# leaxer-ai/leaxer-qwen3-tts

Hardware: AMD Instinct MI355X
Metric: real-time factor (24 kHz audio sec / wall sec), Qwen3-TTS-0.6B (higher is better)
Workload: dtype bf16 weights, fp32 activations/accumulate (codec decoder: fp16 hi/lo split operands, fp32 accumulate)

## Files before the change

### leaxer-qwen3-tts_amd/csrc/q3_common.h

```cpp
#pragma once
#include <hip/hip_runtime.h>
#include <stdint.h>
#include <string>

#include "../../include/q3tts.h"

typedef uint16_t bf16_t;

#define Q3_HIP_CHECK(expr)                                                                         \
    do {                                                                                           \
        hipError_t _e = (expr);                                                                    \
        if (_e != hipSuccess) throw q3::Error(std::string(#expr) + ": " + hipGetErrorString(_e));  \
    } while (0)

namespace q3 {

struct Error {
    std::string msg;
    explicit Error(std::string m) : msg(std::move(m)) {}
};

const char* knob(const char* name);
struct KnobScope {
    bool on = false;
// ... 5 lines not shown
    uint32_t u;
    __builtin_memcpy(&u, &f, 4);
    u = (u + 0x7FFFu + ((u >> 16) & 1u)) >> 16;
    return (bf16_t)u;
}
inline float bf16_to_f32(bf16_t b) {
    uint32_t u = (uint32_t)b << 16;
    float f;
    __builtin_memcpy(&f, &u, 4);
    return f;
}


enum GemvEpi { EPI_STORE = 0, EPI_RESIDUAL = 1, EPI_SWIGLU = 2, EPI_BIAS = 3, EPI_BIAS_SILU = 4, EPI_SLAB = 5, EPI_SLAB2 = 6 };

struct GemvArgs {
    const bf16_t* W = nullptr;
    const bf16_t* W2 = nullptr;
    const float* x = nullptr;
    int ldx = 0;
    const float* gamma = nullptr;
    float eps = 0.f;
    float* xn_out = nullptr;
    int ld_xn = 0;
    const float* bias = nullptr;
    const float* res = nullptr;
    int ldres = 0;
    float* out = nullptr;
    int ldo = 0;
    int M = 0, N = 0, K = 0;
    int epi = EPI_STORE;
    bool nt = false;
    const float* po = nullptr;
    const float* pm = nullptr;
    const float* pl = nullptr;
    int pS = 0, pchunk = 0, pn_new = 1, pslot_offset = 0, pheads = 0, pd = 0;
    const int* ppos_dev = nullptr;
    int ppos_scalar = 0;
    const float* psum = nullptr;
    float* xmid = nullptr;
};
void launch_gemv(const GemvArgs& a, hipStream_t s);
bool gemv_fast_path(const GemvArgs& a);
bool gemv16_ok(const GemvArgs& a);
void launch_gemv16(const GemvArgs& a, hipStream_t s);
void launch_pack_mfma_b(const bf16_t* W, bf16_t* P, int N, int K, hipStream_t s);
size_t packed_mfma_b_elems(int N, int K);
void register_packed_weight(const bf16_t* W, const bf16_t* P);
void unregister_packed_weight(const bf16_t* W);
const bf16_t* find_packed_weight(const bf16_t* W);

struct AttnArgs {
    const float* qkv = nullptr;
    int ld_qkv = 0;
    const float* ssq_in = nullptr; int ssq_nt = 0, ssq_K = 0; float ssq_eps = 0.f;
// ... 116 lines not shown
    float* x_talk = nullptr;
    const float* trailing = nullptr;
    int max_trailing = 0;
    const float* tts_pad = nullptr;
    int32_t* codes = nullptr;
    int max_frames_cap = 0;
    int32_t* talker_pos = nullptr;
    bf16_t* pl_h = nullptr; bf16_t* pl_l = nullptr; int pl_ldp = 0;
    const float* gamma0 = nullptr;
    float* ssq_out = nullptr; int ssq_nt = 0;
    int pl_row_mul = 1, pl_row_add = 0;
    const float* lh = nullptr; int ld_lh = 0;
    unsigned* step_gen = nullptr;
};
void launch_sample(const SampleArgs& a, hipStream_t s);

void launch_gather_rows_bf16(const bf16_t* table, int H, const int64_t* ids_dev, int n, float* out, int ldo, hipStream_t s);
void launch_fill_synth(void* dst, int is_bf16, int64_t n, uint64_t key, float mean, float stddev, hipStream_t s);
void launch_copy_rows(const float* src, int lds, float* dst, int ldd, int rows, int cols, hipStream_t s);
void launch_copy_rows_masked(const float* src, int lds, float* dst, int ldd, int rows, int cols, const int* flags_dev, hipStream_t s);
void launch_bump_u32(unsigned* counter, hipStream_t s);
void launch_count_active(const SlotState* st, int nb, int32_t* out, hipStream_t s);

struct ConvArgs {
    const float* in = nullptr; int T_in = 0, C_in = 0;
    float* out = nullptr;      int T_out = 0, C_out = 0;
    const float* W = nullptr;
    const bf16_t* Wh = nullptr; const bf16_t* Wl = nullptr;
    float w_scale_inv = 1.0f;
    bool w_lo_zero = false, w2_lo_zero = false;
// ... 57 lines not shown
```

### leaxer-qwen3-tts_amd/csrc/q3_decode_kernels.hip

```cpp
#include "q3_common.h"
#include "q3_wave_sort.h"
#include <algorithm>

namespace q3 {

#ifdef Q3_SAMPLE_PROF
__device__ long long g_kernel_prof[32];
void sample_prof_read(long long* out) { (void)hipMemcpyFromSymbol(out, HIP_SYMBOL(g_kernel_prof), sizeof(long long) * 32); }
#define KP_MARK(k) do { if (blockIdx.x == 0 && blockIdx.y == 0 && blockIdx.z == 0 && threadIdx.x == 0) g_kernel_prof[k] = wall_clock64(); } while (0)
#else
#define KP_MARK(k) do { } while (0)
#endif

#define Q3_DPP_XOR1 0xB1
#define Q3_DPP_XOR2 0x4E
#define Q3_DPP_ROR4 0x124
#define Q3_DPP_ROR8 0x128
#define Q3_DPP_BCAST15 0x142
#define Q3_DPP_BCAST31 0x143
template <int CTRL, int ROW_MASK>
static __device__ __forceinline__ float dpp_f(float oldv, float v) {
    return __builtin_bit_cast(float, __builtin_amdgcn_update_dpp(__builtin_bit_cast(int, oldv), __builtin_bit_cast(int, v), CTRL, ROW_MASK, 0xF, false));
}
template <int CTRL, int ROW_MASK>
// ... 391 lines not shown
            if (EPI == EPI_SWIGLU) { s2 = wave_sum(s2); if (lane == m * RW + r) mine2 = s2; }
        }
    KP_MARK(11);
    if (lane < MT * RW) {
        const int m = lane / RW, r = lane % RW, n = n0 + r;
        if (m < M && n < N) {
            float o;
            if (EPI == EPI_STORE) o = mine;
            else if (EPI == EPI_RESIDUAL) o = epi_in + mine;
            else if (EPI == EPI_SWIGLU) o = silu_f(mine) * mine2;
            else if (EPI == EPI_BIAS) o = mine + epi_in;
            else o = silu_f(mine + epi_in);
            a.out[(size_t)m * a.ldo + n] = o;
        }
    }
}

static int gemv1_rw(const GemvArgs& a) {
    int rw = a.N / 1024;
    if (rw < 1) rw = 1;
    if (rw > 4) rw = 4;
    if (a.epi == EPI_SWIGLU && rw > 3) rw = 3;
    if (a.K > 3072 && rw > 2) rw = 2;
    return rw;
}
bool gemv_fast_path(const GemvArgs& a) {
    if (a.M < 1 || a.M > 2) return false;
    if (a.K != 1024 && a.K != 2048 && a.K != 3072 && !(a.K == 6144 && a.M == 1)) return false;
    if (a.ldx % 4 != 0 && !a.po) return false;
    const bool norm = a.gamma != nullptr, comb = a.po != nullptr;
// ... 37 lines not shown
    else if constexpr (NCH <= 6) {
        if (rw == 3) gemv1_launch<MT, NCH, 3>(a, grid, s);
        else gemv1_launch<MT, NCH, 4>(a, grid, s);
    } else throw Error("gemv: K = 6144 fast path takes at most 2 rows per wave");
}
template <int MT>
static void gemv1_nch(const GemvArgs& a, hipStream_t s) {
    if (a.K == 1024) gemv1_rwsel<MT, 2>(a, s);
    else if (a.K == 2048) gemv1_rwsel<MT, 4>(a, s);
    else if (a.K == 3072) gemv1_rwsel<MT, 6>(a, s);
    else if constexpr (MT == 1) gemv1_rwsel<1, 12>(a, s);
    else throw Error("gemv: K = 6144 fast path is single-row");
}

void launch_gemv(const GemvArgs& a0, hipStream_t s) {
    if (gemv_fast_path(a0)) {
        if (a0.M == 1) gemv1_nch<1>(a0, s); else gemv1_nch<2>(a0, s);
        return;
    }
    if (gemv16_ok(a0)) { launch_gemv16(a0, s); return; }
    if (a0.po) throw Error("gemv: attention-partials prologue needs the fast path (combine separately)");
    if (a0.K % 8 != 0 || a0.ldx % 4 != 0) throw Error("gemv: K must be a multiple of 8 and ldx of 4");
    if ((a0.epi == EPI_RESIDUAL || a0.epi == EPI_BIAS || a0.epi == EPI_BIAS_SILU) && a0.gamma) throw Error("gemv: norm+epilogue combination not built");
    if (a0.M <= 0 || a0.N <= 0) return;
    for (int m0 = 0; m0 < a0.M; m0 += 8) {
        GemvArgs a = a0;
        a.M = a0.M - m0 < 8 ? a0.M - m0 : 8;
        a.x = a0.x + (size_t)m0 * a0.ldx;
        a.out = a0.out + (size_t)m0 * a0.ldo;
        if (a0.res) a.res = a0.res + (size_t)m0 * a0.ldres;
// ... 1808 lines not shown
    return draw_small_exact(ei, id0, havei != 0, nk, top_p, u, lane, sb);
}

static __device__ __forceinline__ float kth_largest_of_lanes(float v, int k) {
    const int lane = threadIdx.x & 63;
    const float sorted = wave_sort_desc(v, lane);
    const int r = __builtin_amdgcn_readfirstlane(k) - 1;
    return lane_bcast(sorted, r < 0 ? 0 : (r > 63 ? 63 : r));
}

#ifdef Q3_SAMPLE_PROF
#define SP_MARK(k) do { if (threadIdx.x == 0) g_kernel_prof[k] = wall_clock64(); } while (0)
#else
#define SP_MARK(k) do { } while (0)
#endif
template <bool SLABS, int PW>
__global__ __launch_bounds__(256) void k_sample(const float* plogits, SlotState* pst, int pld, int pV, SampleArgs a) {
    const int b = blockIdx.x, tid = threadIdx.x, lane = tid & 63;
    const int wave = __builtin_amdgcn_readfirstlane(tid >> 6);
    const int V = pV;
    __shared__ float gmax[4][64];
    __shared__ float svw[4][256 + 64];
    __shared__ int svn[4];
    __shared__ float svb[256 + 64];
    __shared__ int cnt_s[SAMP_MAXV / 64];
    __shared__ int cand_idx[SAMP_MAXV + 64];
    __shared__ __attribute__((aligned(16))) float cand_p[SAMP_MAXV + 64];
    __shared__ __attribute__((aligned(16))) float sorted_p[SAMP_MAXV];
    __shared__ int cand_rank[SAMP_MAXV];
    __shared__ __attribute__((aligned(16))) float sb[3][64];
    __shared__ float sh_f[4];
    __shared__ int sh_i[4];

    SP_MARK(0);
    if (a.step_gen != nullptr && b == 0 && tid == 0) *a.step_gen += 1u;
    float temperature = a.temperature, top_p = a.top_p, u = a.u_dev ? a.u_dev[b] : a.u;
    int top_k = a.top_k, suppress = a.suppress, keep_eos = 1;
    int frame = 0;
    SlotState* st = pst ? pst + b : nullptr;
    SlotState sl;
    if (st) {
        const uint4* sp = reinterpret_cast<const uint4*>(st);
        uint4 raw[4] = { sp[0], sp[1], sp[2], sp[3] };
        __builtin_memcpy(&sl, raw, sizeof sl);
    }
    const float* lg = plogits + (size_t)b * pld;
    const int PER = (V + 63) / 64;
    float x[PW];
    if (SLABS) {
        float xp[PW][4];
#pragma unroll
        for (int jj = 0; jj < PW; ++jj) {
            const int i = (wave * PW + jj) * 64 + lane;
#pragma unroll
            for (int sb = 0; sb < 4; ++sb) xp[jj][sb] = lg[(size_t)(sb < a.nslab ? sb : 0) * a.slab_stride + (i < V ? i : V - 1)];
        }
        __builtin_amdgcn_sched_barrier(0);
#pragma unroll
        for (int jj = 0; jj < PW; ++jj) {
            float t = xp[jj][0];
#pragma unroll
            for (int sb = 1; sb < 4; ++sb) t = sb < a.nslab ? t + xp[jj][sb] : t;
            x[jj] = t;
        }
    } else {
#pragma unroll
        for (int jj = 0; jj < PW; ++jj) {
            const int i = (wave * PW + jj) * 64 + lane;
            x[jj] = lg[i < V ? i : V - 1];
        }
    }
    __builtin_amdgcn_sched_barrier(0);
    if (st) {
        if (!sl.active || sl.finished) return;
        if (a.group == 0 && sl.n_frames >= sl.max_frames) { if (tid == 0) st->finished = 1; return; }
        temperature = sl.temperature; top_p = sl.top_p; top_k = sl.top_k;
        frame = sl.n_frames;
        u = rng_uniform_dev(sl.seed, sl.stream_id, (uint32_t)frame, (uint32_t)a.group);
        suppress = a.group == 0;
        keep_eos = !sl.ignore_eos;
    }
    SP_MARK(1);
    const unsigned long long lt_mask = lane == 0 ? 0ull : (~0ull >> (64 - lane));

    const bool use_temp = temperature > 0.0f && temperature != 1.0f;
    float lmax = -INFINITY;
#pragma unroll
    for (int jj = 0; jj < PW; ++jj) {
        const int i = (wave * PW + jj) * 64 + lane;
        float v = x[jj];
// ... 201 lines not shown
                if (pick < 0) {
                    float last = -1.f;
                    for (int c = lane; c < n_kept; c += 64) if (cand_p[c] > 0.f) last = (float)c;
                    last = wave_max(last);
                    pick = last < 0.f ? 0 : (int)last;
                }
                tok = cand_idx[pick];
            }
            if (lane == 0) sh_i[3] = tok;
        }
    }
    __syncthreads();
    tok = sh_i[3];
    SP_MARK(8);

    if (!st) { if (tid == 0) a.token_out[b] = tok; return; }

    if (a.group == 0 && tok == a.eos_id) { if (tid == 0) st->finished = 1; return; }
    if (tid == 0) a.codes[((size_t)b * a.max_frames_cap + frame) * a.n_groups + a.group] = tok;
    const bf16_t* er = a.embed + (size_t)tok * a.H;
    const bool last_group = a.group == a.n_groups - 1;
    const float* text = nullptr;
    if (last_group) text = frame < sl.trailing_len ? a.trailing + ((size_t)b * a.max_trailing + frame) * a.H : a.tts_pad;
    const float* sum_r = a.group != 0 ? a.sum + (size_t)b * a.H : nullptr;
    constexpr int EP_MAX = 2;
    const bool planes = a.pl_h != nullptr && a.x_next != nullptr;
    const float* lh_r = planes && a.lh ? a.lh + (size_t)b * a.ld_lh : nullptr;
    float ss_e = 0.f, ss_l = 0.f;
    for (int h0 = 0; h0 < a.H; h0 += 1024 * EP_MAX) {
        float e[EP_MAX][4], sm[EP_MAX][4], tx[EP_MAX][4], g0[EP_MAX][4], lhv[EP_MAX][4];
#pragma unroll
        for (int it = 0; it < EP_MAX; ++it) {
            int h = h0 + (it * 256 + tid) * 4;
// ... 51 lines not shown
            }
        }
    }
    if (planes) {
        ss_e = wave_sum(ss_e); ss_l = wave_sum(ss_l);
        __syncthreads();
        if (lane == 0) { sh_f[wave] = ss_e; gmax[0][wave] = ss_l; }
        __syncthreads();
        const size_t prow = (size_t)b * a.pl_row_mul + a.pl_row_add;
        if (tid < a.ssq_nt) {
            a.ssq_out[prow * a.ssq_nt + tid] = tid == 0 ? ((sh_f[0] + sh_f[1]) + sh_f[2]) + sh_f[3] : 0.f;
            if (lh_r) a.ssq_out[(prow - 1) * a.ssq_nt + tid] = tid == 0 ? ((gmax[0][0] + gmax[0][1]) + gmax[0][2]) + gmax[0][3] : 0.f;
        }
    }
    if (last_group && tid == 0) {
        st->n_frames = frame + 1;
        a.talker_pos[b] = sl.prompt_len + frame;
    }
}

void launch_sample(const SampleArgs& a, hipStream_t s) {
    if (a.V > SAMP_MAXV) throw Error("sample: vocabulary larger than 4096");
    if (a.nslab < 1 || a.nslab > 4) throw Error("sample: 1..4 logits slabs");
    if (a.pl_h && (a.H > 2048 || a.H % 4 || !a.pl_l || !a.gamma0 || !a.ssq_out || a.ssq_nt < 1 || a.ssq_nt > 256 || a.pl_ldp % 4 || (a.lh && a.pl_row_add < 1)))
        throw Error("sample: bad plane-output arguments");
#define Q3_SAMP(SL, PW_) hipLaunchKernelGGL((k_sample<SL, PW_>), dim3(a.nb), dim3(256), 0, s, a.logits, a.st, a.ld, a.V, a)
    if (a.nslab > 1) { if (a.V <= 2048) Q3_SAMP(true, 8); else if (a.V <= 3072) Q3_SAMP(true, 12); else Q3_SAMP(true, 16); }
    else { if (a.V <= 2048) Q3_SAMP(false, 8); else if (a.V <= 3072) Q3_SAMP(false, 12); else Q3_SAMP(false, 16); }
#undef Q3_SAMP
}

__global__ void k_gather_rows_bf16(const bf16_t* table, int H, const int64_t* ids, float* out, int ldo) {
    const int r = blockIdx.x;
// ... 57 lines not shown
```

### leaxer-qwen3-tts_amd/csrc/q3_engine.cpp

```cpp
#include "q3_engine.h"

#include <algorithm>
#include <atomic>
#include <cmath>
#include <cstdio>
#include <cstdlib>
#include <cstring>

namespace q3 {

static const int64_t TTS_BOS = 151672, TTS_EOS = 151673, TTS_PAD = 151671;
static const int64_t CODEC_BOS = 2149, CODEC_PAD = 2148, CODEC_THINK = 2154, CODEC_NOTHINK = 2155;
static const int64_t CODEC_THINK_BOS = 2156, CODEC_THINK_EOS = 2157, LANG_ENGLISH = 2050;

static uint64_t mix64(uint64_t z) {
    z += 0x9E3779B97F4A7C15ull;
    z = (z ^ (z >> 30)) * 0xBF58476D1CE4E5B9ull;
    z = (z ^ (z >> 27)) * 0x94D049BB133111EBull;
    return z ^ (z >> 31);
}
static uint64_t fnv1a(const std::string& s) {
    uint64_t h = 1469598103934665603ull;
    for (unsigned char ch : s) { h ^= ch; h *= 1099511628211ull; }
    return h;
// ... 137 lines not shown
    if (B < 1 || B > 1024) throw Error("max_batch out of range");
    if (kv_pool_tokens < 0) throw Error("kv_pool_tokens must be >= 0");
    if (c.cp_hidden < 0) throw Error("cp_hidden must be >= 0");
    if (c.cp_hidden == c.hidden) c.cp_hidden = 0;
    if (c.hidden % 8 || c.ffn % 8 || c.text_hidden % 8 || c.cp_ffn % 8 || cp_width() % 8) throw Error("hidden/ffn sizes must be multiples of 8");
    if (c.vocab > 4096 || c.sub_vocab > 4096) throw Error("codec vocabularies larger than 4096 are not supported");
    if (c.n_groups < 2 || c.n_groups > 32) throw Error("n_groups out of range");
    Q3_HIP_CHECK(hipSetDevice(device));
    if (const char* mr = knob("Q3TTS_MFMA_MIN_ROWS")) mfma_min_rows = std::max(3, atoi(mr));
    if (const char* sv = knob("Q3TTS_SEAM")) seam_on = atoi(sv) != 0;
    if (const char* sv = knob("Q3TTS_SEAM_SPIN")) seam_spin = std::max(1, atoi(sv));
    attn_keep_splits = knob("Q3TTS_ATTN_KEEP_SPLITS") != nullptr;
    if (const char* sv = knob("Q3TTS_ATTN_STREAM")) attn_stream = atoi(sv) != 0;
    if (const char* sv = knob("Q3TTS_ATTN_STREAM_ONE")) attn_stream_one = atoi(sv) != 0;
    if (const char* sv = knob("Q3TTS_KVH_OPROJ")) kvh_oproj = atoi(sv) != 0;
    null_stream = getenv("Q3TTS_NULL_STREAM") && getenv("Q3TTS_NULL_STREAM")[0] == '1';
    if (null_stream) { stream = nullptr; flags |= Q3TTS_FLAG_NO_GRAPH; }
    else if (const char* cm = knob("Q3TTS_STREAM_CU_MASK")) {
        const uint32_t pat = (uint32_t)strtoul(cm, nullptr, 16);
        if (pat == 0) throw Error("Q3TTS_STREAM_CU_MASK must be a non-zero hexadecimal CU pattern (a stream with no CU never runs)");
        uint32_t mask[8];
        for (int i = 0; i < 8; ++i) mask[i] = pat;
        Q3_HIP_CHECK(hipExtStreamCreateWithCUMask(&stream, 8, mask));
    }
    else {
        int lo = 0, hi = 0;
        Q3_HIP_CHECK(hipDeviceGetStreamPriorityRange(&lo, &hi));
        Q3_HIP_CHECK(hipStreamCreateWithPriority(&stream, hipStreamNonBlocking, hi));
    }
    Q3_HIP_CHECK(hipEventCreate(&ev0));
// ... 296 lines not shown
    t3 = t1; t3.K = W.ffn;
    t2.seam = 2; t2.epi = EPI_SLAB2; t2.M = M; t2.N = W.ffn; t2.K = W.H; t2.ldo = W.ffn; t2.ldx = ldp; t2.ssq_in = ssq_a_d; t2.ssq_in_nt = NTH;
    t2.seam_cnt = seam_cnt_d; t2.seam_gen = seam_gen_d; t2.oh = pl1h; t2.ol = pl1l; t2.ldp = ldp;
    return gemm_seam_ok(t1, pick_ksplit(AO)) && gemm_seam_ok(t2, ks_q) && gemm_seam_ok(t3, pick_ksplit(W.ffn));
}

bool Engine::run_layers(const DecStack& W, float* x, int ldx, int nb, int n_new, int slot_offset, const int* pos_dev, int pos_scalar,
                        const float* final_gamma, float final_eps, float* final_xn, int final_ld_xn, const int* slot_map) {
    const int M = nb * n_new, QKV = (W.nq + 2 * W.nkv) * W.d, AO = W.nq * W.d;
    const bool mfma = M >= mfma_min_rows && W.H % 128 == 0 && AO % 128 == 0 && W.ffn % 128 == 0 && W.H <= 4096;
    const int ks_q = mfma ? std::min(4, pick_ksplit(W.H)) : 1;
    const int NTH = W.H / 64;
    const bool seam = mfma && seam_applies(W, M, x, ldx, slot_map != nullptr);
    const bool planes_in = planes_in_ready;
    planes_in_ready = false;
    if (planes_in && !seam) throw Error("run_layers: input planes announced without the seam");
    auto seam_counters = [&](int n_tiles) -> unsigned* {
        const size_t need = (size_t)n_tiles * 2 * 16;
        if (seam_cnt_used + need > seam_cnt_words) throw Error("split-K seam: counter buffer too small for this step");
        unsigned* p = seam_cnt_d + seam_cnt_used;
        seam_cnt_used += need;
        return p;
    };
    if (mfma && !planes_in)
        launch_finish(x, ldx, nullptr, 0, 0, 0, W.layers[0].in_norm, W.eps, M, W.H, pl0h, pl0l, ldp, nullptr, 0, stream);
    for (int l = 0; l < W.L; ++l) {
        const DecLayerW& w = W.layers[l];
        if (mfma) {
            GemmArgs g;
            g.W = w.qkv; g.xh = pl0h; g.xl = pl0l; g.ldx = ldp; g.out = qkv_slab_d; g.ldo = QKV; g.M = M; g.N = QKV; g.K = W.H; g.epi = EPI_SLAB; g.nt = W.nt;
            launch_gemm2(g, ks_q, 4, stream);
        } else {
            GemvArgs g;
            g.W = w.qkv; g.x = x; g.ldx = ldx; g.gamma = w.in_norm; g.eps = W.eps; g.out = qkv; g.ldo = QKV;
            g.M = M; g.N = QKV; g.K = W.H; g.epi = EPI_STORE; g.nt = W.nt;
            launch_gemv(g, stream);
        }
        if (!mfma && nb == 1 && pos_dev == nullptr && slot_map == nullptr && W.n_splits == 1 && W.pages_per_slot == 1 && !W.kv_bf16 && !W.kv_round &&
            !(flags & Q3TTS_FLAG_NO_FUSED_CP)) {
            CpAttnOprojArgs f;
            const int ptok = 1 << W.page_shift;
            const size_t coff = (((size_t)slot_offset * W.L + l) * W.nkv) * ptok * W.d;
            f.qkv = qkv; f.ld_qkv = QKV; f.kc = W.kc + coff; f.vc = W.vc + coff; f.page_tokens = ptok; f.base = pos_scalar;
            f.q_norm = w.q_norm; f.k_norm = w.k_norm; f.eps = W.eps; f.rope_cos = W.rope_cos; f.rope_sin = W.rope_sin;
            f.scale = 1.0f / sqrtf((float)W.d); f.nq = W.nq; f.nkv = W.nkv; f.d = W.d; f.W = w.o; f.K = AO; f.N = W.H; f.x = x; f.ldx = ldx;
            if (cp_attn_oproj_ok(f, n_new)) {
                GemvArgs fg;
                fg.W = w.gate; fg.W2 = w.up; fg.x = x; fg.ldx = ldx; fg.gamma = w.post_norm; fg.eps = W.eps; fg.out = act; fg.ldo = W.ffn;
                fg.M = M; fg.N = W.ffn; fg.K = W.H; fg.epi = EPI_SWIGLU; fg.nt = W.nt;
                GemvArgs dg;
                dg.W = w.down; dg.x = act; dg.ldx = W.ffn; dg.res = x; dg.ldres = ldx; dg.out = x; dg.ldo = ldx;
// ... 97 lines not shown
        } else {
            if (direct_rows) { o.po = nullptr; o.pm = nullptr; o.pl = nullptr; }
            else if (!gemv_fast_path(o)) {
                launch_attn_combine(a, stream);
                o.po = nullptr; o.pm = nullptr; o.pl = nullptr;
            }
            launch_gemv(o, stream);
        }
        launch_gemv(f, stream);
        launch_gemv(d, stream);
    }
    return mfma && final_gamma != nullptr;
}

int Engine::head_proj(const bf16_t* Wm, const float* x, int ldx, const float* gamma, float eps, float* xn_out, int ld_xn,
                      float* out, int ldo, int M, int N, int K, bool nt, bool planes_ready, int plane_row0, int plane_row_stride, float* slab_out) {
    if (planes_ready || (M >= mfma_min_rows && K % 128 == 0 && K <= 4096)) {
        if (!planes_ready) {
            launch_finish(const_cast<float*>(x), ldx, nullptr, 0, 0, 0, gamma, eps, M, K, pl0h, pl0l, ldp, xn_out, ld_xn, stream);
            plane_row0 = 0; plane_row_stride = 1;
        }
        GemmArgs g;
        g.W = Wm; g.xh = pl0h + (size_t)plane_row0 * ldp; g.xl = pl0l + (size_t)plane_row0 * ldp; g.ldx = ldp * plane_row_stride;
        g.out = out; g.ldo = ldo; g.M = M; g.N = N; g.K = K; g.epi = EPI_STORE; g.nt = nt;
        if (slab_out != nullptr && M <= 128 && (K == 512 || K == 1024) && ldo % 4 == 0 && !knob("Q3TTS_NO_HEAD_SLABS")) {
            g.out = slab_out; g.epi = EPI_SLAB; g.slab_rows = M;
            launch_gemm2(g, 4, 4, stream);
            return 4;
        }
        launch_gemm2(g, 1, 4, stream);
        return 1;
    }
    GemvArgs g;
    g.W = Wm; g.x = x; g.ldx = ldx; g.gamma = gamma; g.eps = eps; g.xn_out = xn_out; g.ld_xn = ld_xn;
    g.out = out; g.ldo = ldo; g.M = M; g.N = N; g.K = K; g.epi = EPI_STORE; g.nt = nt;
    launch_gemv(g, stream);
    return 1;
}

void Engine::text_project(const int64_t* ids, int n, float* out) {
    if (!finalized) throw Error("weights not finalized");
    if (n <= 0) return;
    const int TH = c.text_hidden, H = c.hidden;
    for (int i = 0; i < n; ++i) if (ids[i] < 0 || ids[i] >= c.text_vocab) throw Error("text id out of range");
    const int np = (n + 15) / 16 * 16;
    if (proj_cap < (size_t)np) {
        sync();
        if (proj_ids_d) (void)hipFree(proj_ids_d);
        if (proj_out_d) (void)hipFree(proj_out_d);
        proj_cap = (size_t)std::max(np, 256);
// ... 312 lines not shown
        float* tr = trailing + toff[u] * H;
        if (nt > 0) memcpy(tr, rows + (size_t)4 * H, (size_t)nt * H * sizeof(float));
        memcpy(tr + (size_t)nt * H, tts_eos, (size_t)H * sizeof(float));
        nt_out[u] = nt + 1;
    }
}

float* Engine::cp_project(float* rows, int ld, int M) {
    if (!cp_projected()) return rows;
    GemvArgs g;
    g.W = cp_proj_w; g.x = rows; g.ldx = ld; g.bias = cp_proj_b; g.out = x_cpp; g.ldo = cp_width(); g.M = M; g.N = cp_width(); g.K = c.hidden; g.epi = EPI_BIAS;
    launch_gemv(g, stream);
    return x_cpp;
}

void Engine::predictor_passes(int nb, const SampleArgs& s0, bool sp0, bool spn, const std::function<void()>& mark) {
    const int H = c.hidden, Hc = cp_width(), SV = c.sub_vocab, G = c.n_groups;
    auto with_planes = [&](SampleArgs& s, int mul, int add, const float* lh, int ld_lh) {
        s.pl_h = pl0h; s.pl_l = pl0l; s.pl_ldp = ldp; s.gamma0 = cp.layers[0].in_norm; s.ssq_out = ssq_b_d; s.ssq_nt = Hc / 64;
        s.pl_row_mul = mul; s.pl_row_add = add; s.lh = lh; s.ld_lh = ld_lh;
    };
    for (int j = 0; j < G - 1; ++j) {
        float* xin = j == 0 ? cp_project(x_cp, H, nb * 2) : cp_project(x_cp1, H, nb);
        bool pr;
        planes_in_ready = j == 0 ? sp0 : spn;
        if (j == 0) pr = run_layers(cp, xin, Hc, nb, 2, 0, nullptr, 0, cp_norm, c.cp_rms_eps);
        else pr = run_layers(cp, xin, Hc, nb, 1, 0, nullptr, j + 1, cp_norm, c.cp_rms_eps);
        const int nsl = head_proj(cp_head[j], j == 0 ? xin + Hc : xin, j == 0 ? 2 * Hc : Hc, cp_norm, c.cp_rms_eps, nullptr, 0, logits_cp, SV, nb, SV, Hc, false,
                                  pr, j == 0 ? 1 : 0, j == 0 ? 2 : 1, trace_d ? nullptr : cp_logit_slab_d);
        mark();
        if (trace_d) launch_copy_rows(logits_cp + (size_t)trace_slot * SV, SV, trace_d + (size_t)(j + 1) * trace_cols, trace_cols, 1, SV, stream);
        SampleArgs s = s0;
        s.logits = nsl > 1 ? cp_logit_slab_d : logits_cp; s.nslab = nsl; s.slab_stride = (size_t)nb * SV;
        s.ld = SV; s.V = SV; s.group = j + 1; s.embed = cp_embed_w[j];
        s.x_next = j + 1 < G - 1 ? x_cp1 : nullptr; s.ld_xnext = H;
        s.pl_h = nullptr; s.lh = nullptr; s.step_gen = nullptr;
        if (spn && s.x_next) with_planes(s, 1, 0, nullptr, 0);
        launch_sample(s, stream);
        mark();
    }
}

void Engine::record_step(int nb) {
    const int H = c.hidden, Hc = cp_width(), V = c.vocab, SV = c.sub_vocab, G = c.n_groups;
    SampleArgs s0;
    s0.logits = logits_t; s0.ld = V; s0.V = V; s0.nb = nb; s0.sup_begin = c.suppress_begin; s0.sup_end = c.suppress_end; s0.eos_id = c.codec_eos;
    s0.group = 0; s0.n_groups = G; s0.st = st_d; s0.embed = codec_embed_w; s0.H = H;
    s0.x_next = x_cp + H; s0.ld_xnext = 2 * H; s0.sum = sum; s0.x_talk = x_talk; s0.trailing = trailing_d; s0.max_trailing = max_trailing;
    s0.tts_pad = tts_pad_d; s0.codes = codes_d; s0.max_frames_cap = max_frames_cap; s0.talker_pos = talker_pos_d;
    size_t mk = 0;
    auto mark = [&]() { if (!stage_ev.empty()) Q3_HIP_CHECK(hipEventRecord(stage_ev[mk++], stream)); };
    struct SeamScope { Engine& e; explicit SeamScope(Engine& en) : e(en) { e.seam_step = true; e.seam_cnt_used = 0; } ~SeamScope() { e.seam_step = false; } } seam_scope(*this);
    s0.step_gen = seam_gen_d;
    mark();
    if (trace_d) launch_copy_rows(logits_t + (size_t)trace_slot * V, V, trace_d, trace_cols, 1, V, stream);
    const bool no_sp = knob("Q3TTS_NO_SAMPLER_PLANES") != nullptr;
    const bool sp_ok = !no_sp && !cp_projected() && H <= 2048 && H % 256 == 0;
    const bool sp0 = sp_ok && seam_applies(cp, nb * 2, x_cp, Hc, false), spn = sp_ok && seam_applies(cp, nb, x_cp1, Hc, false);
    auto with_planes = [&](SampleArgs& s, int mul, int add, const float* lh, int ld_lh) {
        s.pl_h = pl0h; s.pl_l = pl0l; s.pl_ldp = ldp; s.gamma0 = cp.layers[0].in_norm; s.ssq_out = ssq_b_d; s.ssq_nt = Hc / 64;
        s.pl_row_mul = mul; s.pl_row_add = add; s.lh = lh; s.ld_lh = ld_lh;
    };
    if (sp0) with_planes(s0, 2, 1, x_cp, 2 * H);
    launch_sample(s0, stream);
    mark();
    predictor_passes(nb, s0, sp0, spn, mark);
    const bool pr = run_layers(talker, x_talk, H, nb, 1, 0, talker_pos_d, 0, talker_norm, c.rms_eps, x_cp, 2 * H);
    head_proj(codec_head, x_talk, H, talker_norm, c.rms_eps, x_cp, 2 * H, logits_t, V, nb, V, H, true, pr);
    mark();
}

void Engine::stage_profile(int n_steps, double* out) {
    if (!finalized) throw Error("weights not finalized");
    const int nb = nb_in_use(), G = c.n_groups;
    if (nb == 0 || n_steps < 1) throw Error("stage_profile: no armed slot");
    const size_t n_marks = 2 + 2 * (size_t)(G - 1) + 1;
    stage_ev.resize(n_marks);
    for (auto& e : stage_ev) Q3_HIP_CHECK(hipEventCreate(&e));
    double acc[3] = { 0.0, 0.0, 0.0 };
    try {
        for (int i = 0; i < n_steps; ++i) {
            record_step(nb);
            sync();
            for (size_t k = 0; k + 1 < n_marks; ++k) {
// ... 402 lines not shown
```

### leaxer-qwen3-tts_amd/csrc/q3_engine.h

```cpp
#pragma once
#include <functional>
#include <memory>
#include <string>
#include <unordered_map>
#include <vector>

#include "q3_common.h"
#include "q3_kvpool.h"

namespace q3 {

enum TensorKind { TK_W = 0, TK_NORM = 1, TK_BIAS = 2, TK_SCALE = 3, TK_SNAKE = 4 };

struct Tensor {
    std::string name;
    int64_t shape[4] = {0, 0, 0, 0};
    int ndim = 0;
    int kind = TK_W;
    bool bf16 = false;
    void* dev = nullptr;
    int64_t numel = 0;
    float synth_std = 0.02f;
};

// ... 94 lines not shown
    int64_t slot_codec_stream_range(int slot, int a, int b, float* pcm, int64_t cap);
    void slot_codec_stream_reset(int slot);
    void codec_rope_tables(int P);

    void stream_join(hipStream_t caller);
    void stream_fork(hipStream_t caller);
    void talker_prefill_dev(const float* embeds, int nb, int S, const int32_t* lens, float* logits_last, float* last_hidden);
    void talker_decode_dev(const float* embeds, int nb, const uint8_t* active, float* logits, float* last_hidden);
    void code_predictor_dev(const float* last_hidden, const int64_t* code0, int nb, const q3tts_sampling& p, uint64_t seed, uint32_t stream0,
                            uint32_t frame, int32_t* sub);
    void sample_dev(const float* logits, int nb, int V, const q3tts_sampling& p, const float* u, int suppress, int64_t* ids);
    void dev_scratch(int nb);
    float* dev_logits_d = nullptr; int* dev_flags_d = nullptr; int32_t* dev_pos_d = nullptr; int32_t* dev_pos_dummy_d = nullptr;
    SlotState* dev_st_d = nullptr; int32_t* dev_codes_d = nullptr;
    hipEvent_t ev_join = nullptr, ev_fork = nullptr;
    void predictor_passes(int nb, const SampleArgs& s0, bool sp0, bool spn, const std::function<void()>& mark);

    struct SlotInit { int slot = 0; const float* prompt = nullptr; int S = 0; const float* trailing = nullptr; int n_trailing = 0; uint32_t stream_id = 0;
                      int max_frames = 0;
                      int kv_tokens = 0;   };
    void slots_begin(const SlotInit* in, int n, const q3tts_sampling& p, uint64_t seed, int ignore_eos);
    void slot_begin(int slot, const float* prompt, int S, const float* trailing, int n_trailing,
                    const q3tts_sampling& p, uint64_t seed, uint32_t stream_id, int ignore_eos);
    int decode_steps(int n_steps);
    void slot_status(int slot, int* n_frames, int* finished);
    void slot_codes(int slot, int64_t* codes, int cap_frames);
    void slot_logits(int slot, float* logits, float* last_hidden);
    int64_t slot_codec_decode(int slot, float* pcm, int64_t cap);
    void slot_release(int slot);
    void step_bytes(double* wbytes, double* kvbytes);
    void measure_skip_frames(int n);
// ... 50 lines not shown
    std::vector<const bf16_t*> cp_head, cp_embed_w;

    int rows_max = 0, max_trailing = 0, max_frames_cap = 0;
    int mfma_min_rows = 12;
    float *x_talk = nullptr, *qkv = nullptr, *attn = nullptr, *act = nullptr, *logits_t = nullptr, *logits_cp = nullptr;
    float *x_cp = nullptr, *x_cp1 = nullptr, *sum = nullptr, *xp = nullptr, *hn = nullptr, *logits_p = nullptr;
    float *trailing_d = nullptr, *tts_pad_d = nullptr, *text_tmp = nullptr, *text_tmp2 = nullptr;
    int64_t* ids_d = nullptr;
    bf16_t *pl0h = nullptr, *pl0l = nullptr, *pl1h = nullptr, *pl1l = nullptr;
    int ldp = 0;
    float* slab_d = nullptr;
    float* gu_slab_d = nullptr;
    float* cp_logit_slab_d = nullptr;
    float* qkv_slab_d = nullptr;
    float *oproj_part_d = nullptr, *xmid_d = nullptr;
    bool kvh_oproj = true;
    unsigned* seam_cnt_d = nullptr; size_t seam_cnt_words = 0, seam_cnt_used = 0;
    unsigned* seam_gen_d = nullptr;
    float *ssq_a_d = nullptr, *ssq_b_d = nullptr;
    bool seam_step = false;
    bool seam_on = true;
    bool attn_stream = true;
    bool attn_stream_one = true;
    bool attn_keep_splits = false;
    int seam_spin = 512;
    int32_t* codes_d = nullptr;
    int32_t* codes_scratch_d = nullptr;
    int32_t* talker_pos_d = nullptr;
    int* slot_map_d = nullptr;
    float* logits_g = nullptr;
// ... 2 lines not shown
    int32_t* active_d = nullptr;
    int32_t* active_h = nullptr;
    int64_t* tok_d = nullptr;
    hipEvent_t ev0 = nullptr, ev1 = nullptr;
    std::unordered_map<int, hipGraphExec_t> graphs;

    void* dmalloc(size_t bytes);
    bool run_layers(const DecStack& W, float* x, int ldx, int nb, int n_new, int slot_offset, const int* pos_dev, int pos_scalar,
                    const float* final_gamma = nullptr, float final_eps = 0.f, float* final_xn = nullptr, int final_ld_xn = 0,
                    const int* slot_map = nullptr);
    void record_step(int nb);
    bool seam_applies(const DecStack& W, int M, float* x, int ldx, bool has_slot_map) const;
    bool planes_in_ready = false;
    int head_proj(const bf16_t* Wm, const float* x, int ldx, const float* gamma, float eps, float* xn_out, int ld_xn,
                  float* out, int ldo, int M, int N, int K, bool nt, bool planes_ready = false, int plane_row0 = 0, int plane_row_stride = 1,
                  float* slab_out = nullptr);
    int nb_in_use() const;
    void sync();
};

}
```

Baseline: 38.28.

## Fold token sampler into the next stack's first QKV GEMV kernel

For single-slot decode, the sampling kernel is no longer launched separately. Every workgroup of the first-layer QKV GEMV redundantly recomputes the sample and builds the embedding input row in registers, while only block 0 writes the shared state. The frame counter commit moves to the codec-head GEMV epilogue. This removes one kernel launch and one dependency boundary per sampling pass, at the cost of redundant sampling work in every block and extra shared memory and registers in the GEMV.

Result: faster. 38.81, median of 6 (+1.4%).

```diff
diff --git a/leaxer-qwen3-tts_amd/csrc/q3_common.h b/leaxer-qwen3-tts_amd/csrc/q3_common.h
--- a/leaxer-qwen3-tts_amd/csrc/q3_common.h
+++ b/leaxer-qwen3-tts_amd/csrc/q3_common.h
@@ -43,6 +43,7 @@
 
 enum GemvEpi { EPI_STORE = 0, EPI_RESIDUAL = 1, EPI_SWIGLU = 2, EPI_BIAS = 3, EPI_BIAS_SILU = 4, EPI_SLAB = 5, EPI_SLAB2 = 6 };
 
+struct SlotState;
 struct GemvArgs {
     const bf16_t* W = nullptr;
     const bf16_t* W2 = nullptr;
@@ -68,6 +69,7 @@
     int ppos_scalar = 0;
     const float* psum = nullptr;
     float* xmid = nullptr;
+    SlotState* st_commit = nullptr;
 };
 void launch_gemv(const GemvArgs& a, hipStream_t s);
 bool gemv_fast_path(const GemvArgs& a);
@@ -214,6 +216,8 @@
     unsigned* step_gen = nullptr;
 };
 void launch_sample(const SampleArgs& a, hipStream_t s);
+bool gemv_samp_ok(const GemvArgs& g, const SampleArgs& s);
+void launch_gemv_samp(const GemvArgs& g, const SampleArgs& s, hipStream_t st);
 
 void launch_gather_rows_bf16(const bf16_t* table, int H, const int64_t* ids_dev, int n, float* out, int ldo, hipStream_t s);
 void launch_fill_synth(void* dst, int is_bf16, int64_t n, uint64_t key, float mean, float stddev, hipStream_t s);
diff --git a/leaxer-qwen3-tts_amd/csrc/q3_decode_kernels.hip b/leaxer-qwen3-tts_amd/csrc/q3_decode_kernels.hip
--- a/leaxer-qwen3-tts_amd/csrc/q3_decode_kernels.hip
+++ b/leaxer-qwen3-tts_amd/csrc/q3_decode_kernels.hip
@@ -429,6 +429,10 @@
             a.out[(size_t)m * a.ldo + n] = o;
         }
     }
+    if (EPI == EPI_STORE && a.st_commit != nullptr && blockIdx.x == 0 && threadIdx.x == 0) {
+        SlotState* st = a.st_commit;
+        if (st->active && !st->finished) st->n_frames = st->n_frames + 1;
+    }
 }
 
 static int gemv1_rw(const GemvArgs& a) {
@@ -496,6 +500,7 @@
 }
 
 void launch_gemv(const GemvArgs& a0, hipStream_t s) {
+    if (a0.st_commit && (a0.epi != EPI_STORE || !gemv_fast_path(a0))) throw Error("gemv: the frame commit needs the single-pass EPI_STORE kernel");
     if (gemv_fast_path(a0)) {
         if (a0.M == 1) gemv1_nch<1>(a0, s); else gemv1_nch<2>(a0, s);
         return;
@@ -2334,39 +2339,31 @@
 #else
 #define SP_MARK(k) do { } while (0)
 #endif
+struct SampSmem {
+    float gmax[4][64];
+    float svw[4][256 + 64];
+    int svn[4];
+    float svb[256 + 64];
+    int cnt_s[SAMP_MAXV / 64];
+    int cand_idx[SAMP_MAXV + 64];
+    __attribute__((aligned(16))) float cand_p[SAMP_MAXV + 64];
+    __attribute__((aligned(16))) float sorted_p[SAMP_MAXV];
+    int cand_rank[SAMP_MAXV];
+    __attribute__((aligned(16))) float sb[3][64];
+    float sh_f[4];
+    int sh_i[4];
+};
+
 template <bool SLABS, int PW>
-__global__ __launch_bounds__(256) void k_sample(const float* plogits, SlotState* pst, int pld, int pV, SampleArgs a) {
-    const int b = blockIdx.x, tid = threadIdx.x, lane = tid & 63;
-    const int wave = __builtin_amdgcn_readfirstlane(tid >> 6);
-    const int V = pV;
-    __shared__ float gmax[4][64];
-    __shared__ float svw[4][256 + 64];
-    __shared__ int svn[4];
-    __shared__ float svb[256 + 64];
-    __shared__ int cnt_s[SAMP_MAXV / 64];
-    __shared__ int cand_idx[SAMP_MAXV + 64];
-    __shared__ __attribute__((aligned(16))) float cand_p[SAMP_MAXV + 64];
-    __shared__ __attribute__((aligned(16))) float sorted_p[SAMP_MAXV];
-    __shared__ int cand_rank[SAMP_MAXV];
-    __shared__ __attribute__((aligned(16))) float sb[3][64];
-    __shared__ float sh_f[4];
-    __shared__ int sh_i[4];
-
-    SP_MARK(0);
-    if (a.step_gen != nullptr && b == 0 && tid == 0) *a.step_gen += 1u;
-    float temperature = a.temperature, top_p = a.top_p, u = a.u_dev ? a.u_dev[b] : a.u;
-    int top_k = a.top_k, suppress = a.suppress, keep_eos = 1;
-    int frame = 0;
-    SlotState* st = pst ? pst + b : nullptr;
-    SlotState sl;
+static __device__ __forceinline__ void samp_load(const float* plogits, const SlotState* st, int pld, int V, const SampleArgs& a, int b, int wave, int lane,
+                                                 float (&x)[PW], SlotState& sl, float& u) {
+    u = a.u_dev ? a.u_dev[b] : a.u;
     if (st) {
         const uint4* sp = reinterpret_cast<const uint4*>(st);
         uint4 raw[4] = { sp[0], sp[1], sp[2], sp[3] };
         __builtin_memcpy(&sl, raw, sizeof sl);
     }
     const float* lg = plogits + (size_t)b * pld;
-    const int PER = (V + 63) / 64;
-    float x[PW];
     if (SLABS) {
         float xp[PW][4];
 #pragma unroll
@@ -2390,10 +2387,20 @@
             x[jj] = lg[i < V ? i : V - 1];
         }
     }
-    __builtin_amdgcn_sched_barrier(0);
+}
+
+template <int PW>
+static __device__ __forceinline__ int samp_draw(float (&x)[PW], SlotState* st, const SlotState& sl, int V, const SampleArgs& a, float u, int tid, int wave,
+                                                int lane, SampSmem& S, bool writer, int& frame) {
+    auto& gmax = S.gmax; auto& svw = S.svw; auto& svn = S.svn; auto& svb = S.svb; auto& cnt_s = S.cnt_s; auto& cand_idx = S.cand_idx;
+    auto& cand_p = S.cand_p; auto& sorted_p = S.sorted_p; auto& cand_rank = S.cand_rank; auto& sb = S.sb; auto& sh_f = S.sh_f; auto& sh_i = S.sh_i;
+    const int PER = (V + 63) / 64;
+    float temperature = a.temperature, top_p = a.top_p;
+    int top_k = a.top_k, suppress = a.suppress, keep_eos = 1;
+    frame = 0;
     if (st) {
-        if (!sl.active || sl.finished) return;
-        if (a.group == 0 && sl.n_frames >= sl.max_frames) { if (tid == 0) st->finished = 1; return; }
+        if (!sl.active || sl.finished) return -1;
+        if (a.group == 0 && sl.n_frames >= sl.max_frames) { if (writer && tid == 0) st->finished = 1; return -1; }
         temperature = sl.temperature; top_p = sl.top_p; top_k = sl.top_k;
         frame = sl.n_frames;
         u = rng_uniform_dev(sl.seed, sl.stream_id, (uint32_t)frame, (uint32_t)a.group);
@@ -2625,9 +2632,13 @@
     tok = sh_i[3];
     SP_MARK(8);
 
-    if (!st) { if (tid == 0) a.token_out[b] = tok; return; }
-
-    if (a.group == 0 && tok == a.eos_id) { if (tid == 0) st->finished = 1; return; }
+    if (st && a.group == 0 && tok == a.eos_id) { if (writer && tid == 0) st->finished = 1; return -1; }
+    return tok;
+}
+
+static __device__ __forceinline__ void samp_epilogue(const SampleArgs& a, SlotState* st, const SlotState& sl, int b, int frame, int tok, int tid, int wave,
+                                                     int lane, SampSmem& S, bool commit_frame) {
+    auto& gmax = S.gmax; auto& sh_f = S.sh_f;
     if (tid == 0) a.codes[((size_t)b * a.max_frames_cap + frame) * a.n_groups + a.group] = tok;
     const bf16_t* er = a.embed + (size_t)tok * a.H;
     const bool last_group = a.group == a.n_groups - 1;
@@ -2709,9 +2720,178 @@
         }
     }
     if (last_group && tid == 0) {
-        st->n_frames = frame + 1;
+        if (commit_frame) st->n_frames = frame + 1;
         a.talker_pos[b] = sl.prompt_len + frame;
     }
+}
+
+template <bool SLABS, int PW>
+__global__ __launch_bounds__(256) void k_sample(const float* plogits, SlotState* pst, int pld, int pV, SampleArgs a) {
+    const int b = blockIdx.x, tid = threadIdx.x, lane = tid & 63;
+    const int wave = __builtin_amdgcn_readfirstlane(tid >> 6);
+    __shared__ SampSmem S;
+
+    SP_MARK(0);
+    if (a.step_gen != nullptr && b == 0 && tid == 0) *a.step_gen += 1u;
+    SlotState* st = pst ? pst + b : nullptr;
+    SlotState sl;
+    float x[PW], u;
+    samp_load<SLABS, PW>(plogits, st, pld, pV, a, b, wave, lane, x, sl, u);
+    __builtin_amdgcn_sched_barrier(0);
+    int frame;
+    const int tok = samp_draw<PW>(x, st, sl, pV, a, u, tid, wave, lane, S, true, frame);
+    if (!st) { if (tid == 0) a.token_out[b] = tok; return; }
+    if (tok < 0) return;
+    samp_epilogue(a, st, sl, b, frame, tok, tid, wave, lane, S, true);
+}
+
+template <int MT, int PW>
+__global__ __launch_bounds__(256) void k_gemv1_samp(const float* plogits, SlotState* pst, const bf16_t* pW, const float* px, const float* pgamma,
+                                                    int pV, int pN, int pldx, int pnt, SampleArgs sa, GemvArgs a) {
+    constexpr int NCH = 2, RW = 4, K = NCH * 512;
+    const int tid = threadIdx.x, lane = tid & 63;
+    const int wave = __builtin_amdgcn_readfirstlane(tid >> 6);
+    const int n0 = (blockIdx.x * 4 + wave) * RW;
+    const int N = pN;
+    const bool writer = blockIdx.x == 0;
+    __shared__ SampSmem S;
+
+    if (sa.step_gen != nullptr && writer && tid == 0) *sa.step_gen += 1u;
+    SlotState sl;
+    float xl[PW], u;
+    samp_load<false, PW>(plogits, pst, sa.ld, pV, sa, 0, wave, lane, xl, sl, u);
+    __builtin_amdgcn_sched_barrier(0);
+    uint4 w[RW][NCH];
+#pragma unroll
+    for (int r = 0; r < RW; ++r) {
+        const int n = n0 + r < N ? n0 + r : N - 1;
+#pragma unroll
+        for (int c = 0; c < NCH; ++c) w[r][c] = ldw_rt(pW + (size_t)n * K + c * 512 + lane * 8, pnt != 0);
+    }
+    __builtin_amdgcn_sched_barrier(0);
+    float xv[MT][NCH][8], g[NCH][8];
+#pragma unroll
+    for (int m = 0; m + 1 < MT; ++m)
+#pragma unroll
+        for (int c = 0; c < NCH; ++c) {
+            const float* xr = px + (size_t)m * pldx + c * 512 + lane * 8;
+            const float4 x0 = *reinterpret_cast<const float4*>(xr);
+            const float4 x1 = *reinterpret_cast<const float4*>(xr + 4);
+            xv[m][c][0] = x0.x; xv[m][c][1] = x0.y; xv[m][c][2] = x0.z; xv[m][c][3] = x0.w;
+            xv[m][c][4] = x1.x; xv[m][c][5] = x1.y; xv[m][c][6] = x1.z; xv[m][c][7] = x1.w;
+        }
+#pragma unroll
+    for (int c = 0; c < NCH; ++c) {
+        const float4 g0 = *reinterpret_cast<const float4*>(pgamma + c * 512 + lane * 8);
+        const float4 g1 = *reinterpret_cast<const float4*>(pgamma + c * 512 + lane * 8 + 4);
+        g[c][0] = g0.x; g[c][1] = g0.y; g[c][2] = g0.z; g[c][3] = g0.w; g[c][4] = g1.x; g[c][5] = g1.y; g[c][6] = g1.z; g[c][7] = g1.w;
+    }
+    __builtin_amdgcn_sched_barrier(0);
+    int frame = 0;
+    const int tok = samp_draw<PW>(xl, pst, sl, pV, sa, u, tid, wave, lane, S, writer, frame);
+    constexpr int ML = MT - 1;
+    if (tok >= 0) {
+        const bool last_group = sa.group == sa.n_groups - 1;
+        const bool need_sum = last_group || (writer && wave == 1 && sa.group != 0);
+        const bf16_t* er = sa.embed + (size_t)tok * sa.H;
+        const float* text = last_group ? (frame < sl.trailing_len ? sa.trailing + (size_t)frame * sa.H : sa.tts_pad) : nullptr;
+        uint4 e[NCH];
+        float4 sm[NCH][2], tx[NCH][2];
+#pragma unroll
+        for (int c = 0; c < NCH; ++c) {
+            const int k = c * 512 + lane * 8;
+            e[c] = *reinterpret_cast<const uint4*>(er + k);
+            if (need_sum) { sm[c][0] = *reinterpret_cast<const float4*>(sa.sum + k); sm[c][1] = *reinterpret_cast<const float4*>(sa.sum + k + 4); }
+            if (last_group) { tx[c][0] = *reinterpret_cast<const float4*>(text + k); tx[c][1] = *reinterpret_cast<const float4*>(text + k + 4); }
+        }
+        __builtin_amdgcn_sched_barrier(0);
+        float ev[NCH][8], sv[NCH][8];
+#pragma unroll
+        for (int c = 0; c < NCH; ++c) {
+            const uint32_t eu[4] = { e[c].x, e[c].y, e[c].z, e[c].w };
+            const float smf[8] = { sm[c][0].x, sm[c][0].y, sm[c][0].z, sm[c][0].w, sm[c][1].x, sm[c][1].y, sm[c][1].z, sm[c][1].w };
+            const float txf[8] = { tx[c][0].x, tx[c][0].y, tx[c][0].z, tx[c][0].w, tx[c][1].x, tx[c][1].y, tx[c][1].z, tx[c][1].w };
+#pragma unroll
+            for (int j = 0; j < 8; ++j) {
+                ev[c][j] = (j & 1) ? bf_hi(eu[j >> 1]) : bf_lo(eu[j >> 1]);
+                sv[c][j] = sa.group == 0 ? ev[c][j] : (need_sum ? smf[j] + ev[c][j] : 0.f);
+                xv[ML][c][j] = last_group ? sv[c][j] + txf[j] : ev[c][j];
+            }
+        }
+        if (writer) {
+            if (tid == 0) sa.codes[(size_t)frame * sa.n_groups + sa.group] = tok;
+            if (last_group && tid == 0) sa.talker_pos[0] = sl.prompt_len + frame;
+            auto store_row = [&](float* orow, const float (&src)[NCH][8]) {
+#pragma unroll
+                for (int c = 0; c < NCH; ++c) {
+                    float* o = orow + c * 512 + lane * 8;
+                    *reinterpret_cast<float4*>(o) = make_float4(src[c][0], src[c][1], src[c][2], src[c][3]);
+                    *reinterpret_cast<float4*>(o + 4) = make_float4(src[c][4], src[c][5], src[c][6], src[c][7]);
+                }
+            };
+            if (wave == 0 && sa.x_next) store_row(sa.x_next, ev);
+            if (wave == 1 && !last_group) store_row(sa.sum, sv);
+            if (wave == 2 && last_group) store_row(sa.x_talk, xv[ML]);
+        }
+    } else {
+#pragma unroll
+        for (int c = 0; c < NCH; ++c) {
+            const float* xr = px + (size_t)ML * pldx + c * 512 + lane * 8;
+            const float4 x0 = *reinterpret_cast<const float4*>(xr);
+            const float4 x1 = *reinterpret_cast<const float4*>(xr + 4);
+            xv[ML][c][0] = x0.x; xv[ML][c][1] = x0.y; xv[ML][c][2] = x0.z; xv[ML][c][3] = x0.w;
+            xv[ML][c][4] = x1.x; xv[ML][c][5] = x1.y; xv[ML][c][6] = x1.z; xv[ML][c][7] = x1.w;
+        }
+    }
+#pragma unroll
+    for (int m = 0; m < MT; ++m) {
+        float ss = 0.f;
+#pragma unroll
+        for (int c = 0; c < NCH; ++c)
+#pragma unroll
+            for (int j = 0; j < 8; ++j) ss = fmaf(xv[m][c][j], xv[m][c][j], ss);
+        ss = wave_sum(ss);
+        const float inv = 1.0f / sqrtf(ss / (float)K + a.eps);
+#pragma unroll
+        for (int c = 0; c < NCH; ++c)
+#pragma unroll
+            for (int j = 0; j < 8; ++j) xv[m][c][j] = g[c][j] * (xv[m][c][j] * inv);
+    }
+    float mine = 0.f;
+#pragma unroll
+    for (int m = 0; m < MT; ++m)
+#pragma unroll
+        for (int r = 0; r < RW; ++r) {
+            float s1 = 0.f;
+#pragma unroll
+            for (int c = 0; c < NCH; ++c) {
+                const uint32_t wu[4] = { w[r][c].x, w[r][c].y, w[r][c].z, w[r][c].w };
+#pragma unroll
+                for (int j = 0; j < 4; ++j) { s1 = fmaf(xv[m][c][2 * j], bf_lo(wu[j]), s1); s1 = fmaf(xv[m][c][2 * j + 1], bf_hi(wu[j]), s1); }
+            }
+            s1 = wave_sum(s1);
+            if (lane == m * RW + r) mine = s1;
+        }
+    if (lane < MT * RW) {
+        const int m = lane / RW, r = lane % RW, n = n0 + r;
+        if (n < N) a.out[(size_t)m * a.ldo + n] = mine;
+    }
+}
+
+bool gemv_samp_ok(const GemvArgs& g, const SampleArgs& s) {
+    const int pw_v = g.M == 1 ? 2048 : 3072;
+    return gemv_fast_path(g) && g.gamma && g.epi == EPI_STORE && !g.psum && !g.po && !g.xn_out && g.K == 1024 && gemv1_rw(g) == 4 &&
+           s.st && s.nb == 1 && s.nslab == 1 && !s.pl_h && s.H == g.K && s.V <= pw_v && (g.M == 1 || s.V > 2048) && s.embed && s.codes && s.sum;
+}
+
+void launch_gemv_samp(const GemvArgs& g, const SampleArgs& s, hipStream_t st) {
+    if (!gemv_samp_ok(g, s)) throw Error("gemv_samp: shape not built (b = 1, K = 1024, four rows per wave, one logits slab)");
+    const bool last = s.group == s.n_groups - 1;
+    if ((last ? s.x_talk : s.x_next) != g.x + (size_t)(g.M - 1) * g.ldx || (last && (!s.talker_pos || !s.trailing || !s.tts_pad)))
+        throw Error("gemv_samp: the consumer's input row is not the sampler's output row");
+    const int grid = (g.N + 15) / 16;
+    if (g.M == 1) hipLaunchKernelGGL((k_gemv1_samp<1, 8>), dim3(grid), dim3(256), 0, st, s.logits, s.st, g.W, g.x, g.gamma, s.V, g.N, g.ldx, (int)g.nt, s, g);
+    else hipLaunchKernelGGL((k_gemv1_samp<2, 12>), dim3(grid), dim3(256), 0, st, s.logits, s.st, g.W, g.x, g.gamma, s.V, g.N, g.ldx, (int)g.nt, s, g);
 }
 
 void launch_sample(const SampleArgs& a, hipStream_t s) {
diff --git a/leaxer-qwen3-tts_amd/csrc/q3_engine.cpp b/leaxer-qwen3-tts_amd/csrc/q3_engine.cpp
--- a/leaxer-qwen3-tts_amd/csrc/q3_engine.cpp
+++ b/leaxer-qwen3-tts_amd/csrc/q3_engine.cpp
@@ -175,6 +175,7 @@
     if (const char* sv = knob("Q3TTS_ATTN_STREAM")) attn_stream = atoi(sv) != 0;
     if (const char* sv = knob("Q3TTS_ATTN_STREAM_ONE")) attn_stream_one = atoi(sv) != 0;
     if (const char* sv = knob("Q3TTS_KVH_OPROJ")) kvh_oproj = atoi(sv) != 0;
+    if (const char* sv = knob("Q3TTS_SAMPLE_FOLD")) sample_fold = atoi(sv) != 0;
     null_stream = getenv("Q3TTS_NULL_STREAM") && getenv("Q3TTS_NULL_STREAM")[0] == '1';
     if (null_stream) { stream = nullptr; flags |= Q3TTS_FLAG_NO_GRAPH; }
     else if (const char* cm = knob("Q3TTS_STREAM_CU_MASK")) {
@@ -501,6 +502,9 @@
     const bool seam = mfma && seam_applies(W, M, x, ldx, slot_map != nullptr);
     const bool planes_in = planes_in_ready;
     planes_in_ready = false;
+    const bool fold = fold_armed;
+    fold_armed = false;
+    if (fold && mfma) throw Error("run_layers: a folded sampler needs the GEMV QKV projection");
     if (planes_in && !seam) throw Error("run_layers: input planes announced without the seam");
     auto seam_counters = [&](int n_tiles) -> unsigned* {
         const size_t need = (size_t)n_tiles * 2 * 16;
@@ -521,7 +525,8 @@
             GemvArgs g;
             g.W = w.qkv; g.x = x; g.ldx = ldx; g.gamma = w.in_norm; g.eps = W.eps; g.out = qkv; g.ldo = QKV;
             g.M = M; g.N = QKV; g.K = W.H; g.epi = EPI_STORE; g.nt = W.nt;
-            launch_gemv(g, stream);
+            if (l == 0 && fold) launch_gemv_samp(g, fold_args, stream);
+            else launch_gemv(g, stream);
         }
         if (!mfma && nb == 1 && pos_dev == nullptr && slot_map == nullptr && W.n_splits == 1 && W.pages_per_slot == 1 && !W.kv_bf16 && !W.kv_round &&
             !(flags & Q3TTS_FLAG_NO_FUSED_CP)) {
@@ -649,8 +654,10 @@
 }
 
 int Engine::head_proj(const bf16_t* Wm, const float* x, int ldx, const float* gamma, float eps, float* xn_out, int ld_xn,
-                      float* out, int ldo, int M, int N, int K, bool nt, bool planes_ready, int plane_row0, int plane_row_stride, float* slab_out) {
+                      float* out, int ldo, int M, int N, int K, bool nt, bool planes_ready, int plane_row0, int plane_row_stride, float* slab_out,
+                      SlotState* commit_st) {
     if (planes_ready || (M >= mfma_min_rows && K % 128 == 0 && K <= 4096)) {
+        if (commit_st) throw Error("head_proj: the frame commit rides on the GEMV head");
         if (!planes_ready) {
             launch_finish(const_cast<float*>(x), ldx, nullptr, 0, 0, 0, gamma, eps, M, K, pl0h, pl0l, ldp, xn_out, ld_xn, stream);
             plane_row0 = 0; plane_row_stride = 1;
@@ -668,7 +675,7 @@
     }
     GemvArgs g;
     g.W = Wm; g.x = x; g.ldx = ldx; g.gamma = gamma; g.eps = eps; g.xn_out = xn_out; g.ld_xn = ld_xn;
-    g.out = out; g.ldo = ldo; g.M = M; g.N = N; g.K = K; g.epi = EPI_STORE; g.nt = nt;
+    g.out = out; g.ldo = ldo; g.M = M; g.N = N; g.K = K; g.epi = EPI_STORE; g.nt = nt; g.st_commit = commit_st;
     launch_gemv(g, stream);
     return 1;
 }
@@ -1011,7 +1018,7 @@
     return x_cpp;
 }
 
-void Engine::predictor_passes(int nb, const SampleArgs& s0, bool sp0, bool spn, const std::function<void()>& mark) {
+void Engine::predictor_passes(int nb, const SampleArgs& s0, bool sp0, bool spn, const std::function<void()>& mark, bool fold) {
     const int H = c.hidden, Hc = cp_width(), SV = c.sub_vocab, G = c.n_groups;
     auto with_planes = [&](SampleArgs& s, int mul, int add, const float* lh, int ld_lh) {
         s.pl_h = pl0h; s.pl_l = pl0l; s.pl_ldp = ldp; s.gamma0 = cp.layers[0].in_norm; s.ssq_out = ssq_b_d; s.ssq_nt = Hc / 64;
@@ -1033,7 +1040,8 @@
         s.x_next = j + 1 < G - 1 ? x_cp1 : nullptr; s.ld_xnext = H;
         s.pl_h = nullptr; s.lh = nullptr; s.step_gen = nullptr;
         if (spn && s.x_next) with_planes(s, 1, 0, nullptr, 0);
-        launch_sample(s, stream);
+        if (fold) { fold_args = s; fold_armed = true; }
+        else launch_sample(s, stream);
         mark();
     }
 }
@@ -1059,12 +1067,27 @@
         s.pl_row_mul = mul; s.pl_row_add = add; s.lh = lh; s.ld_lh = ld_lh;
     };
     if (sp0) with_planes(s0, 2, 1, x_cp, 2 * H);
-    launch_sample(s0, stream);
+    const bool fold = sample_fold && !sp0 && !spn && trace_d == nullptr && stage_ev.empty() && fold_fits(nb);
+    if (fold) { fold_args = s0; fold_armed = true; }
+    else launch_sample(s0, stream);
     mark();
-    predictor_passes(nb, s0, sp0, spn, mark);
+    predictor_passes(nb, s0, sp0, spn, mark, fold);
     const bool pr = run_layers(talker, x_talk, H, nb, 1, 0, talker_pos_d, 0, talker_norm, c.rms_eps, x_cp, 2 * H);
-    head_proj(codec_head, x_talk, H, talker_norm, c.rms_eps, x_cp, 2 * H, logits_t, V, nb, V, H, true, pr);
+    head_proj(codec_head, x_talk, H, talker_norm, c.rms_eps, x_cp, 2 * H, logits_t, V, nb, V, H, true, pr, 0, 1, nullptr, fold ? st_d : nullptr);
     mark();
+    if (fold_armed) { fold_armed = false; throw Error("record_step: a folded sampler was not consumed"); }
+}
+
+bool Engine::fold_fits(int nb) const {
+    if (nb != 1 || cp_projected() || mfma_min_rows <= 2) return false;
+    auto fits = [&](const DecStack& W, int M, int V) {
+        GemvArgs g;
+        g.W = W.layers[0].qkv; g.x = x_cp; g.ldx = W.H; g.gamma = W.layers[0].in_norm; g.M = M; g.N = (W.nq + 2 * W.nkv) * W.d; g.K = W.H; g.epi = EPI_STORE;
+        SampleArgs s;
+        s.st = st_d; s.nb = 1; s.H = c.hidden; s.V = V; s.embed = codec_embed_w; s.codes = codes_d; s.sum = sum;
+        return W.L > 0 && gemv_samp_ok(g, s);
+    };
+    return fits(cp, 2, c.vocab) && fits(cp, 1, c.sub_vocab) && fits(talker, 1, c.sub_vocab);
 }
 
 void Engine::stage_profile(int n_steps, double* out) {
diff --git a/leaxer-qwen3-tts_amd/csrc/q3_engine.h b/leaxer-qwen3-tts_amd/csrc/q3_engine.h
--- a/leaxer-qwen3-tts_amd/csrc/q3_engine.h
+++ b/leaxer-qwen3-tts_amd/csrc/q3_engine.h
@@ -132,7 +132,7 @@
     float* dev_logits_d = nullptr; int* dev_flags_d = nullptr; int32_t* dev_pos_d = nullptr; int32_t* dev_pos_dummy_d = nullptr;
     SlotState* dev_st_d = nullptr; int32_t* dev_codes_d = nullptr;
     hipEvent_t ev_join = nullptr, ev_fork = nullptr;
-    void predictor_passes(int nb, const SampleArgs& s0, bool sp0, bool spn, const std::function<void()>& mark);
+    void predictor_passes(int nb, const SampleArgs& s0, bool sp0, bool spn, const std::function<void()>& mark, bool fold = false);
 
     struct SlotInit { int slot = 0; const float* prompt = nullptr; int S = 0; const float* trailing = nullptr; int n_trailing = 0; uint32_t stream_id = 0;
                       int max_frames = 0;
@@ -213,6 +213,10 @@
     float* cp_logit_slab_d = nullptr;
     float* qkv_slab_d = nullptr;
     float *oproj_part_d = nullptr, *xmid_d = nullptr;
+    bool sample_fold = true;
+    SampleArgs fold_args;
+    bool fold_armed = false;
+    bool fold_fits(int nb) const;
     bool kvh_oproj = true;
     unsigned* seam_cnt_d = nullptr; size_t seam_cnt_words = 0, seam_cnt_used = 0;
     unsigned* seam_gen_d = nullptr;
@@ -245,7 +249,7 @@
     bool planes_in_ready = false;
     int head_proj(const bf16_t* Wm, const float* x, int ldx, const float* gamma, float eps, float* xn_out, int ld_xn,
                   float* out, int ldo, int M, int N, int K, bool nt, bool planes_ready = false, int plane_row0 = 0, int plane_row_stride = 1,
-                  float* slab_out = nullptr);
+                  float* slab_out = nullptr, SlotState* commit_st = nullptr);
     int nb_in_use() const;
     void sync();
 };
```
